# claforte/RayTracingWeekend.jl

Measured on AMD Instinct MI355X. Metric: Msamples/s (pixels x spp) on scene_random_spheres 1920x1080, higher is better.
Workload: dtype f32

## Files before the change

### raytracingweekend.jl_amd/csrc/rtw_host.hpp

```cpp
#pragma once
#pragma GCC visibility push(default)
#include "../../include/rtw_hip.h"
#pragma GCC visibility pop

#include <hip/hip_runtime.h>

#include <algorithm>
#include <atomic>
#include <cmath>
#include <cstdarg>
#include <cstddef>
#include <cstdint>
#include <cstdio>
#include <cstdlib>
#include <cstring>
#include <initializer_list>
#include <limits>
#include <map>
#include <memory>
#include <mutex>
#include <string>
#include <thread>
#include <type_traits>
#include <vector>
// ... 1 lines not shown
#pragma GCC visibility push(hidden)

#include "rtw_layout.hpp"

namespace rtw { struct DevCounters; }


struct rtw_scene_dev {
    int device;
    int is_f64;
    int n, n_pad;
    void *geom, *mat0, *mat1;
    void *scan;
    void *mf_ops;
    int mf_blocks;
    float mf_sc, mf_sigma2, mf_oo_keep, mf_o1_coef, mf_o_max;
    int n_huge, huge[2];
    void *p_mf_ops, *p_geom, *p_mat0, *p_mat1;
    unsigned short *p_orig;
    int p_alias, p_n, p_n_pad, p_mf_blocks, p_huge[2];
    void *c_mf_ops, *c_mf_box;
    float c_glo[3], c_ghi[3];
    int c_mf_blocks;
    float c_grid[6];
    int c_n_inlane, c_inlane[8];
    void *c_bound, *c_exact, *c_mat0, *c_mat1;
    unsigned short *c_orig;
    int c_groups_pad, c_big;
    double c_cs[3], c_rs;
    uint64_t content_hash;
};
// ... 285 lines not shown
```

### raytracingweekend.jl_amd/csrc/rtw_launch.hip

```cpp
#include "rtw_scene_view.hpp"
#include "rtw_kernels.hpp"
#include "rtw_instances.hpp"
#ifdef RTW_WITH_POOL
#include "rtw_pool.hpp"
template <typename T> using pool_kern_t = void (*)(rtw::KParams, rtw::Camera<T>, rtw::DevScene<T>, T *, rtw::DevCounters *);
#endif

namespace rtwh {

void make_udiv(unsigned d, unsigned *m, unsigned *s) {
    if (d <= 1) { *m = 0; *s = 0x80000000u; return; }
    unsigned l = 0;
    while ((1ull << l) < d) ++l;
    *m = (unsigned)((((1ull << l) - d) << 32) / d + 1);
    *s = l - 1;
}

struct PoolChoice { bool use = false; const void *kern = nullptr; size_t lds = 0; int block_threads = 256, blocks_per_cu = 0; };
template <typename T>
static int choose_pool(const DeviceCtx *ctx, const rtw_scene_dev *scene, const rtw_params *p, int cs, bool eligible, bool phase_profile, PoolChoice *pool) {
#ifdef RTW_WITH_POOL
    static const bool env_pool = aid_flag("RTW_POOL");
    if constexpr (sizeof(T) == 4) {
        pool->lds = rtw::pool_fixed_lds_bytes<T, RTW_POOL_W, RTW_POOL_R>() + rtw::pool_scene_lds_bytes<T>(scene->n, scene->n_pad);
// ... 238 lines not shown
    } else if (aid_env("RTW_PHASE_PROFILE")) {
        double tot = 0;
        for (int k = 0; k < 6; ++k) tot += (double)c.phase[k];
        fprintf(stderr, "[rtw phase profile] wave-cycles: pull %.1f%%  sample+scatter finish %.1f%%  scan-pass1/level1 %.1f%%  extract/level2 %.1f%%  resolve %.1f%%  shade %.1f%%  (total %.3g)\n",
                100 * c.phase[0] / tot, 100 * c.phase[1] / tot, 100 * c.phase[2] / tot, 100 * c.phase[4] / tot,
                100 * c.phase[5] / tot, 100 * c.phase[3] / tot, tot);
        if (c.phase[8])
            fprintf(stderr, "[rtw phase profile] lane loop: %llu wave-iterations, lane utilisation at the scan %.2f %% (%llu lanes with a ray), %.2f %% of the iterations without any ray; "
                            "lane-iterations lost at batch boundaries %.2f %% (pool short) + %.2f %% (no usable batch)\n", (unsigned long long)c.phase[8],
                    100.0 * (double)c.phase[9] / (64.0 * (double)c.phase[8]), (unsigned long long)c.phase[9], 100.0 * (double)c.phase[10] / (double)c.phase[8],
                    100.0 * (double)c.phase[11] / (64.0 * (double)c.phase[8]), 100.0 * (double)c.phase[12] / (64.0 * (double)c.phase[8]));
        if (c.phase[8]) {
            fprintf(stderr, "[rtw phase counts] per wave-iteration:");
            static const char *nm[32] = {0, 0, 0, 0, 0, 0, "blocks_without_candidate", "blocks", "iterations", "lanes_with_ray", "iterations_without_ray", "takers_pool_short", "takers_unserved",
                                         "list_entries", "exact_test_rounds", "exact_tests", "reject_trials", "R_executed", "H1_executed", "H1_rounds", "A_executed", "jobs_stored", "batches_set_up",
                                         "H2_executed", "B_executed", "F_normalize_executed", "sign_collections", "blocks_recording", "explode_iterations", "reject_trials_3_draws", 0, 0};
            for (int k = 6; k < 32; ++k) if (nm[k]) fprintf(stderr, " %s=%.4f", nm[k], (double)c.phase[k] / (double)c.phase[8]);
            fprintf(stderr, "\n");
        }
        if (c.phase[8] && c.phase[13])
            fprintf(stderr, "[rtw phase profile] pass 2: %.1f list entries, %.2f exact-test rounds and %.1f exact tests per wave-iteration (lanes busy in a round: %.1f %%)\n",
                    (double)c.phase[13] / (double)c.phase[8], (double)c.phase[14] / (double)c.phase[8], (double)c.phase[15] / (double)c.phase[8], 100.0 * (double)c.phase[15] / (64.0 * (double)c.phase[14]));
        if (c.phase[7])
            fprintf(stderr, "[rtw phase profile] matrix-pipe scan: %.1f%% of the (wave, block of 32 spheres) evaluations found no candidate in any lane (%llu of %llu)\n",
                    100.0 * (double)c.phase[6] / (double)c.phase[7], (unsigned long long)c.phase[6], (unsigned long long)c.phase[7]);
    }
    if (r->ctr_bytes == sizeof(rtw::DevCounters) && c.end_hist[0] == 0xdeadbeefu) {
        fprintf(stderr, "[rtw pool watchdog]");
        for (int k = 1; k <= 113; ++k) fprintf(stderr, " %u", c.end_hist[k]);
        fprintf(stderr, "\n");
    }
// ... 32 lines not shown
```

### raytracingweekend.jl_amd/csrc/rtw_probes.hpp

```cpp
#pragma once

#ifdef RTW_DUP_OPERANDS
#define RTW_PROBE_OPERANDS_TWICE()                                                                                                          \
    {                                                                                                                                       \
        float ox2 = ox, oy2 = oy, oz2 = oz, dx2_ = dx, dy2_ = dy, dz2_ = dz;                                                                \
        __asm__ volatile("" : "+v"(ox2), "+v"(oy2), "+v"(oz2), "+v"(dx2_), "+v"(dy2_), "+v"(dz2_));                                         \
        const float q_ = __builtin_fmaf(oz2, dz2_, __builtin_fmaf(oy2, dy2_, ox2 * dx2_));                                                  \
        const float oo_ = __builtin_fmaf(oz2, oz2, __builtin_fmaf(oy2, oy2, ox2 * ox2));                                                    \
        const float o1_ = (__builtin_fabsf(ox2) + __builtin_fabsf(oy2)) + __builtin_fabsf(oz2);                                             \
        const float oop_ = __builtin_fmaf(oo_, w.mf_oo_keep, -(w.mf_o1_coef * o1_));                                                        \
        const float tq_ = w.mf_sigma2 * __builtin_fmaf(q_, q_, -oop_);                                                                      \
        const float fp_[3] = {__builtin_fmaf(-q_, dx2_, ox2) * zs2, __builtin_fmaf(-q_, dy2_, oy2) * zs2, __builtin_fmaf(-q_, dz2_, oz2) * zs2}; \
        const float ax_ = dx2_ * z2, ay_ = dy2_ * z2, az_ = dz2_ * z2;                                                                      \
        const float fq_[6] = {ax_ * dx2_, ay_ * dy2_, az_ * dz2_, (ax_ + ax_) * dy2_, (ax_ + ax_) * dz2_, (ay_ + ay_) * dz2_};              \
        unsigned sq_[6], sp_[3];                                                                                                            \
        for (int k = 0; k < 6; ++k) sq_[k] = split_f16(fq_[k]);                                                                             \
        for (int k = 0; k < 3; ++k) sp_[k] = split_f16(fp_[k]);                                                                             \
        const float tx_ = ok ? tq_ : tx;                                                                                                    \
        const _Float16 t1_ = (_Float16)(tx_ * (1.0f / 32768.0f));                                                                           \
        const unsigned x23_ = split_f16((tx_ - 32768.0f * (float)t1_) * (1.0f / 16.0f));                                                    \
        const unsigned a0[8] = {dup(sq_[0]), cat(sq_[0], sq_[1]), sq_[1], dup(sq_[2]), sq_[5], dup(sp_[0]), cat(sp_[0], sp_[1]), sp_[1]};   \
        const unsigned a1[8] = {cat(sq_[2], sq_[3]), sq_[3], dup(sq_[4]), cat(sq_[4], sq_[5]), dup(sp_[2]), cat(sp_[2], sb),                \
                                ss | ((unsigned)__builtin_bit_cast(unsigned short, t1_) << 16), x23_};                                      \
        for (int k = 0; k < 8; ++k) {                                                                                                       \
            const auto sw2 = __builtin_amdgcn_permlane32_swap(a0[k], a1[k], false, false);                                                  \
            __asm__ volatile("" :: "v"(sw2[0]), "v"(sw2[1]));                                                                               \
        }                                                                                                                                   \
    }
#else
#define RTW_PROBE_OPERANDS_TWICE()
#endif

#ifdef RTW_PROBE_NO_MFMA
#define RTW_PROBE_FILTER_PAIR_REPLACED(a1, a2, b1, b2)                                                                                      \
    {                                                                                                                                       \
        rtw_f16v Wn = {-1, -1, -1, -1, -1, -1, -1, -1, -1, -1, -1, -1, -1, -1, -1, -1};                                                     \
        const uint4 u1 = __builtin_bit_cast(uint4, b1), u2 = __builtin_bit_cast(uint4, b2);                                                 \
        __asm__ volatile("" :: "v"(a1.x), "v"(a1.y), "v"(a1.z), "v"(a1.w), "v"(a2.x), "v"(a2.y), "v"(a2.z), "v"(a2.w));                     \
// ... 70 lines not shown
```

### raytracingweekend.jl_amd/csrc/rtw_scan.hpp

```cpp
#pragma once
#include "rtw_path.hpp"

namespace rtw {

#define RTW_SPHERE_WORD 32
#define RTW_SPHERE_TAIL 8
__host__ __device__ inline int scene_geom_alloc(int n, int n_pad) {
    const int a = n_pad + RTW_SPHERE_TAIL, b = ((n + 31) / 32) * 32;
    return a > b ? a : b;
}
template <typename T> struct DevScene {
    const float *scan;
    const typename Vec4<T>::type *geom;
    const typename Vec4<T>::type *mat0;
    const typename Vec4<T>::type *mat1;
    int n, n_pad;
    const uint4 *mf_ops;
    int mf_blocks;
    float mf_sc;
    float mf_sigma2;
    float mf_oo_keep;
    float mf_o1_coef;
    float mf_o_max;
    int n_huge, huge[2];
    int numerics;
    const unsigned short *orig;
};

#define RTW_LIST_CAP 16
#define RTW_LDS_SCENE_MAX_BYTES (24 * 1024)

__device__ __forceinline__ uint32_t sign_word(float x) { return __float_as_uint(x); }
__device__ __forceinline__ uint32_t sign_word(double x) { return (uint32_t)((uint64_t)__double_as_longlong(x) >> 32); }

#ifndef RTW_SCAN_PRIO
#define RTW_SCAN_PRIO 1
#endif
template <typename T> struct ScanGroup;
// ... 175 lines not shown
```

### raytracingweekend.jl_amd/csrc/rtw_scan_mfma.hpp

```cpp
#pragma once
#include "rtw_scan.hpp"
#include "rtw_cull_tables.hpp"
#include "rtw_probes.hpp"

namespace rtw {

#define RTW_PAIR_CAP 512
typedef _Float16 rtw_h8 __attribute__((ext_vector_type(8)));
typedef float rtw_f16v __attribute__((ext_vector_type(16)));

__host__ __device__ inline int cull_tab_words(int blocks) { return ((blocks + 31) / 32 > 0 ? (blocks + 31) / 32 : 1) * RTW_CULL_TAB_WORDS; }
struct CullGrid {
    float inv[3], off[3];
};

struct MfmaCull {
    const uint4 *ops;
    const float *box;
    int blocks;
    float cs[3], rs;
    const void *mat0;
    float glo[3], ghi[3];
    int n_huge;
    int n_exact;
// ... 17 lines not shown
__device__ __forceinline__ float lane_get(float v, unsigned src_lane) {
    return __int_as_float(__builtin_amdgcn_ds_bpermute((int)(src_lane << 2), __float_as_int(v)));
}
__device__ __forceinline__ double lane_get(double v, unsigned src_lane) {
    const long long b = __double_as_longlong(v);
    const unsigned lo = (unsigned)__builtin_amdgcn_ds_bpermute((int)(src_lane << 2), (int)(unsigned)b);
    const unsigned hi = (unsigned)__builtin_amdgcn_ds_bpermute((int)(src_lane << 2), (int)(unsigned)((unsigned long long)b >> 32));
    return __longlong_as_double((long long)(((unsigned long long)hi << 32) | lo));
}

#ifndef RTW_INLANE_FILTER
#define RTW_INLANE_FILTER 1
#endif
#ifndef RTW_PRECHECK_GROUPS
#define RTW_PRECHECK_GROUPS 1
#endif
#ifndef RTW_SCAN_SKIP
#define RTW_SCAN_SKIP 1
#endif

struct NoOrig {};
template <typename T, bool WITH_R, typename SRC, typename ORIG = NoOrig, typename SINK = NoSink>
__device__ __forceinline__ void test_singles(int num, SRC src, [[maybe_unused]] const typename Vec4<T>::type *rad, V3<T> o, V3<T> d, T tmin, const WaveScratch &ws, const unsigned *singles, unsigned n, unsigned lane, ORIG orig, unsigned *prof, [[maybe_unused]] SINK sink = SINK()) {
    constexpr bool CULLED = !__is_same(ORIG, NoOrig);
    using V4 = typename Vec4<T>::type;
    for (unsigned p0 = 0; p0 < n; p0 += 64u) {
        const unsigned p = p0 + lane;
        const bool valid = p < n;
        const unsigned e = singles[valid ? p : 0u];
        if (prof) { prof[0] += 1u; prof[1] += (unsigned)__popcll(__ballot(valid)); }
// ... 62 lines not shown
    __builtin_amdgcn_wave_barrier();
}

template <typename T, typename SRC, typename RAD, typename ORIG = NoOrig, typename SINK = NoSink>
__device__ __forceinline__ void resolve_pairs(int num, SRC src, RAD rad, V3<T> o, V3<T> d, T tmin, const WaveScratch &ws, unsigned n, unsigned lane, ORIG orig = ORIG(), unsigned *prof = nullptr, SINK sink = SINK()) {
    if (num == NUM_REFERENCE_FMA2) resolve_pairs_impl<T, true>(num, src, rad(), o, d, tmin, ws, n, lane, orig, prof, sink);
    else resolve_pairs_impl<T, false>(num, src, nullptr, o, d, tmin, ws, n, lane, orig, prof, sink);
}

template <typename T, typename SRC, typename ORIG = NoOrig, typename CLK = NoClock, typename SINK = NoSink, bool VOTE = !__is_same(ORIG, NoOrig)>
__device__ __forceinline__ int hit_world_mfma(const DevScene<T> &w, SRC src, V3<T> o, V3<T> d, bool has_ray, T tmin, T &t_hit,
                                              const WaveScratch &ws, unsigned lane, CLK &&clk = NoClock(),
                                              const MfmaCull *mc = nullptr, ORIG orig = ORIG(), SINK sink = SINK()) {
    constexpr bool HAS_ORIG = !__is_same(ORIG, NoOrig);
    constexpr bool CULLED = VOTE;
    static_assert(HAS_ORIG || !VOTE, "the group cull's order comes with its index array");
    auto rad = [&]() -> const typename Vec4<T>::type * { if constexpr (CULLED) return (const typename Vec4<T>::type *)mc->mat0; else return w.mat0; };
    const float ox = (float)o.x, oy = (float)o.y, oz = (float)o.z, dx = (float)d.x, dy = (float)d.y, dz = (float)d.z;
    const float s2 = __builtin_fmaf(dz, dz, __builtin_fmaf(dy, dy, dx * dx));
    const float oinf = __builtin_fmaxf(__builtin_fmaxf(__builtin_fabsf(ox), __builtin_fabsf(oy)), __builtin_fabsf(oz));
    const bool ok = has_ray && s2 <= 1.0009f && oinf <= w.mf_o_max;
    if constexpr (SINK::on()) { if (has_ray) sink.ray(lane, ok, w.mf_sc); }
    const float q = __builtin_fmaf(oz, dz, __builtin_fmaf(oy, dy, ox * dx));
    const float oo = __builtin_fmaf(oz, oz, __builtin_fmaf(oy, oy, ox * ox));
    const float o1 = (__builtin_fabsf(ox) + __builtin_fabsf(oy)) + __builtin_fabsf(oz);
    const float oop = __builtin_fmaf(oo, w.mf_oo_keep, -(w.mf_o1_coef * o1));
    const float tq = w.mf_sigma2 * __builtin_fmaf(q, q, -oop);
    const float z = ok ? 1.0f : 0.0f, z2 = z + z, zs2 = z2 * w.mf_sc;
    const float fp[3] = {__builtin_fmaf(-q, dx, ox) * zs2, __builtin_fmaf(-q, dy, oy) * zs2, __builtin_fmaf(-q, dz, oz) * zs2};
    const float dx2 = dx * z2, dy2 = dy * z2, dz2 = dz * z2;
// ... 45 lines not shown
        mine = (cells_ok ? mine : 0u) | t[flag_word];
        mine |= (unsigned)__builtin_amdgcn_update_dpp(0, (int)mine, 0xB1, 0xf, 0xf, true);
        mine |= (unsigned)__builtin_amdgcn_update_dpp(0, (int)mine, 0x4E, 0xf, 0xf, true);
        mine |= (unsigned)__builtin_amdgcn_update_dpp(0, (int)mine, 0x141, 0xf, 0xf, true);
        mine |= (unsigned)__builtin_amdgcn_update_dpp(0, (int)mine, 0x140, 0xf, 0xf, true);
        v0_ = (unsigned)__builtin_amdgcn_readlane((int)mine, 0) | (unsigned)__builtin_amdgcn_readlane((int)mine, 16);
        v1_ = (unsigned)__builtin_amdgcn_readlane((int)mine, 32) | (unsigned)__builtin_amdgcn_readlane((int)mine, 48);
    };
    uint4 A1 = {0u, 0u, 0u, 0u}, A2 = {0u, 0u, 0u, 0u};
    auto fetch = [&](int b) {
        typedef unsigned u4 __attribute__((ext_vector_type(4)));
        const __attribute__((address_space(1))) u4 *q = (const __attribute__((address_space(1))) u4 *)pa_of(b);
        __asm__("" : "+s"(q));
        A1 = __builtin_bit_cast(uint4, q[(size_t)lane]); A2 = __builtin_bit_cast(uint4, q[(size_t)lane + 64u]);
    };
    if constexpr (!CULLED) fetch(0);
    unsigned sq[6], sp[3];
#pragma unroll
    for (int k = 0; k < 6; ++k) sq[k] = split_f16(fq[k]);
#pragma unroll
    for (int k = 0; k < 3; ++k) sp[k] = split_f16(fp[k]);
    const _Float16 t1 = (_Float16)(tx * (1.0f / 32768.0f));
    const float trem = tx - 32768.0f * (float)t1;
    const unsigned x23 = split_f16(trem * (1.0f / 16.0f));
    const unsigned sb = ok ? 0x7800u : 0u, ss = ok ? 0x4c00u : 0u;
    auto dup = [](unsigned v) { return __builtin_amdgcn_perm(v, v, 0x01000100u); };
    auto cat = [](unsigned a, unsigned b) { return __builtin_amdgcn_alignbit(b, a, 16); };
    const unsigned g0[8] = {dup(sq[0]), cat(sq[0], sq[1]), sq[1], dup(sq[2]),
                            sq[5], dup(sp[0]), cat(sp[0], sp[1]), sp[1]};
    const unsigned g1[8] = {cat(sq[2], sq[3]), sq[3], dup(sq[4]), cat(sq[4], sq[5]),
                            dup(sp[2]), cat(sp[2], sb), ss | ((unsigned)__builtin_bit_cast(unsigned short, t1) << 16), x23};
    unsigned h0[8], h1[8];
#pragma unroll
    for (int k = 0; k < 8; ++k) {
        const auto sw = __builtin_amdgcn_permlane32_swap(g0[k], g1[k], false, false);
        h0[k] = sw[0]; h1[k] = sw[1];
    }
    RTW_PROBE_OPERANDS_TWICE();
    rtw_h8 B1[2], B2[2];
    {
        const uint4 q10 = {h0[0], h0[1], h0[2], h0[3]}, q11 = {h1[0], h1[1], h1[2], h1[3]};
        const uint4 q20 = {h0[4], h0[5], h0[6], h0[7]}, q21 = {h1[4], h1[5], h1[6], h1[7]};
        B1[0] = __builtin_bit_cast(rtw_h8, q10); B1[1] = __builtin_bit_cast(rtw_h8, q11);
        B2[0] = __builtin_bit_cast(rtw_h8, q20); B2[1] = __builtin_bit_cast(rtw_h8, q21);
    }
    const unsigned lane_const = lane << 16;
// ... 112 lines not shown
            }
            return any;
        };
        [[maybe_unused]] auto eval = [&](const rtw_f16v &Wv, unsigned &bits) {
#pragma unroll
            for (int r = 0; r < 16; ++r) bits = __builtin_amdgcn_alignbit(bits, __float_as_uint(Wv[r]), 31);
        };
        auto filter_pair = [&](const uint4 &a1, const uint4 &a2, const rtw_h8 &b1, const rtw_h8 &b2) -> rtw_f16v {
            RTW_PROBE_FILTER_PAIR_REPLACED(a1, a2, b1, b2);
            rtw_f16v Wp = __builtin_amdgcn_mfma_f32_32x32x16_f16(__builtin_bit_cast(rtw_h8, a1), b1, zero, 0, 0, 0);
            Wp = __builtin_amdgcn_mfma_f32_32x32x16_f16(__builtin_bit_cast(rtw_h8, a2), b2, Wp, 0, 0, 0);
            RTW_PROBE_FILTER_PAIR_AGAIN(Wp, a1, a2, b1, b2);
            return Wp;
        };
        unsigned long long some0 = 0ull, some1 = 0ull;
        if (!CULLED || do_half0) {
            rtw_f16v Wv = filter_pair(A1, A2, B1[0], B2[0]);
            RTW_PROBE_EVAL_TWICE(Wv);
            some0 = collect(Wv, bits);
        }
        if (!CULLED || do_half1) {
            rtw_f16v Wv = filter_pair(A1, A2, B1[1], B2[1]);
            __builtin_amdgcn_sched_barrier(0);
            fetch(blk);
            __builtin_amdgcn_sched_barrier(0);
            RTW_PROBE_EVAL_TWICE(Wv);
            some1 = collect(Wv, bits);
        } else {
            fetch(blk);
        }
        clk.lap(2);
        if constexpr (!CULLED) clk.count(7, 1u);
        if (RTW_SCAN_SKIP && !(some0 | some1)) {
            if constexpr (!CULLED) clk.count(6, 1u);
        } else {
        unsigned long long got1 = some1;
        __asm__("" : "+s"(got1));
        const unsigned m = ~bits << (got1 ? 0u : 16u);
        if constexpr (!CULLED) { if (!__any(m != 0u)) clk.count(6, 1u); }
        const unsigned long long act = __ballot(m != 0u);
        clk.count(27, 1u);
        if (total + 64u > ws.cap) {
            clk.lap(4);
            if constexpr (SINK::on()) sink.flush(lane, RTW_FLUSH_A);
// ... 36 lines not shown
```

### raytracingweekend.jl_amd/csrc/rtw_scene.hip

```cpp
#include "rtw_scene_view.hpp"
#include "rtw_cull_tables.hpp"
#include "rtw_plain_layout.hpp"

namespace rtwh {

template <typename SceneT>
void kd_split(const SceneT *s, std::vector<int> &ids, int lo, int hi, std::vector<std::vector<int>> &groups) {
    const int cnt = hi - lo;
    if (cnt <= RTW_CULL_GS) {
        if (cnt > 0) groups.emplace_back(ids.begin() + lo, ids.begin() + hi);
        return;
    }
    double mn[3] = {1e300, 1e300, 1e300}, mx[3] = {-1e300, -1e300, -1e300};
    for (int k = lo; k < hi; ++k) {
        const double c[3] = {(double)s->cx[ids[k]], (double)s->cy[ids[k]], (double)s->cz[ids[k]]};
        for (int a = 0; a < 3; ++a) { mn[a] = std::min(mn[a], c[a]); mx[a] = std::max(mx[a], c[a]); }
    }
    int ax = 0;
    for (int a = 1; a < 3; ++a) if (mx[a] - mn[a] > mx[ax] - mn[ax]) ax = a;
    const int unit = cnt > 2 * RTW_CULL_GS ? 2 * RTW_CULL_GS : RTW_CULL_GS;
    int half = ((cnt / 2 + unit - 1) / unit) * unit;
    if (half >= cnt) half = cnt - 1;
    auto key = [&](int i) { return ax == 0 ? (double)s->cx[i] : ax == 1 ? (double)s->cy[i] : (double)s->cz[i]; };
    std::nth_element(ids.begin() + lo, ids.begin() + lo + half, ids.begin() + hi, [&](int a, int b) { return key(a) < key(b); });
// ... 155 lines not shown

template <typename T, typename V4>
int build_mfma_operands(const std::vector<V4> &geom, int n, rtw_scene_dev *h, void **ops_out, int *blocks_out, int n_skip, const int *skip, int n_rows) {
    *ops_out = nullptr; *blocks_out = 0;
    if (n <= 0) return 0;
    auto live = [&](int i) { return i < n && (double)geom[i].w > -1e29; };
    if (n_rows < 0) n_rows = n;
    auto in_filter = [&](int i) { if (!live(i) || i >= n_rows) return false; for (int k = 0; k < n_skip; ++k) if (skip[k] == i) return false; return true; };
    double emax = 0;
    for (int i = 0; i < n; ++i) {
        if (!live(i)) continue;
        const double r = std::sqrt(std::fabs((double)geom[i].w));
        emax = std::max(emax, std::max(std::max(std::fabs((double)(float)geom[i].x), std::fabs((double)(float)geom[i].y)),
                                       std::max(std::fabs((double)(float)geom[i].z), r)));
    }
    if (!(emax > 0) || !std::isfinite(emax)) return 0;
    int ex = 0;
    (void)std::frexp(emax, &ex);
    if (ex > 40 || ex < -40) return 0;
    const double sc = std::ldexp(1.0, 8 - ex), sig2 = sc * sc;
    const double phi_c = std::ldexp(1.0, -25) / sc, phi_k = std::ldexp(1.0, -20) / sig2;
    const double A_S = std::ldexp(1.0, -17), A_r = std::ldexp(12.0, -22);
    auto split = [](double x, unsigned &p1, unsigned &p2) {
        const float xf = (float)x;
        const _Float16 h1 = (_Float16)xf;
        const _Float16 h2 = (_Float16)(xf - (float)h1);
        unsigned short b1, b2;
        memcpy(&b1, &h1, 2); memcpy(&b2, &h2, 2);
        p1 = b1; p2 = b2;
    };
    const int nb = (n_rows + 31) / 32;
    std::vector<uint4> ops((size_t)(nb + 1) * 128);
    for (int blk = 0; blk <= nb; ++blk)
        for (int lane = 0; lane < 64; ++lane) {
            const int i = lane & 31, H = lane >> 5;
            const int sph = blk * 32 + 16 * ((i >> 2) & 1) + (((i >> 3) << 2) | (i & 3));
            double fq[6] = {0, 0, 0, 0, 0, 0}, fl[3] = {0, 0, 0};
            double kx = -1073741824.0;
            if (in_filter(sph)) {
                const double cx = (double)(float)geom[sph].x, cy = (double)(float)geom[sph].y, cz = (double)(float)geom[sph].z;
                const double r2 = (double)geom[sph].w, c2 = cx * cx + cy * cy + cz * cz;
                const double Gs = 1.02 * ((2 * A_S + A_r) * c2 + A_r * r2 + 9 * phi_c * (std::fabs(cx) + std::fabs(cy) + std::fabs(cz)) + 1.5 * phi_k);
                kx = (r2 - c2 + Gs) * sig2;
                const double hs = 0.5 * sig2;
                fq[0] = cx * cx * hs; fq[1] = cy * cy * hs; fq[2] = cz * cz * hs; fq[3] = cx * cy * hs; fq[4] = cx * cz * hs; fq[5] = cy * cz * hs;
                fl[0] = cx * sc; fl[1] = cy * sc; fl[2] = cz * sc;
            }
            unsigned q1[6], q2[6], l1[3], l2[3];
            for (int k = 0; k < 6; ++k) split(fq[k], q1[k], q2[k]);
            for (int k = 0; k < 3; ++k) split(fl[k], l1[k], l2[k]);
            const _Float16 k1 = (_Float16)(float)(kx / 32768.0);
            const double rem = (kx - 32768.0 * (double)(float)k1) / 16.0;
            _Float16 k2 = (_Float16)(float)rem;
            if ((double)(float)k2 < rem) { unsigned short b; memcpy(&b, &k2, 2); b = (unsigned short)((float)k2 >= 0.0f ? b + 1 : b - 1); memcpy(&k2, &b, 2); }
            unsigned short kb1, kb2;
            memcpy(&kb1, &k1, 2); memcpy(&kb2, &k2, 2);
            auto pk = [](unsigned lo, unsigned hi) { return (lo & 0xffffu) | (hi << 16); };
            uint4 m1, m2;
            if (H == 0) {
                m1 = uint4{pk(q1[0], q2[0]), pk(q1[0], q1[1]), pk(q2[1], q1[1]), pk(q1[2], q2[2])};
                m2 = uint4{pk(q2[5], q1[5]), pk(l1[0], l2[0]), pk(l1[0], l1[1]), pk(l2[1], l1[1])};
            } else {
                m1 = uint4{pk(q1[2], q1[3]), pk(q2[3], q1[3]), pk(q1[4], q2[4]), pk(q1[4], q1[5])};
                m2 = uint4{pk(l1[2], l2[2]), pk(l1[2], kb1), pk(kb2, 0x7800u), 0x4c004c00u};
            }
            ops[(size_t)blk * 128 + lane] = m1;
            ops[(size_t)blk * 128 + 64 + lane] = m2;
        }
    HIP_TRY(hipMalloc(ops_out, ops.size() * sizeof(uint4)));
    HIP_TRY(hipMemcpy(*ops_out, ops.data(), ops.size() * sizeof(uint4), hipMemcpyHostToDevice));
    *blocks_out = nb;
    h->mf_sc = (float)sc; h->mf_sigma2 = (float)sig2;
    float keep = (float)(1.0 - 1.02 * 2 * A_S);
    if ((double)keep > 1.0 - 1.02 * 2 * A_S) keep = std::nextafter(keep, 0.0f);
    h->mf_oo_keep = keep;
    float coef = (float)(1.02 * 9 * phi_c);
    if ((double)coef < 1.02 * 9 * phi_c) coef = std::nextafter(coef, INFINITY);
    h->mf_o1_coef = coef;
    h->mf_o_max = (float)(std::ldexp(1.0, 13) / sc);
    return 0;
}

template <typename T, typename V4>
int build_plain(const std::vector<V4> &geom, const std::vector<V4> &mat0, const std::vector<V4> &mat1, int n, rtw_scene_dev *h) {
    if (!h->mf_ops) return 0;
    static const bool keep_env = aid_env("RTW_PLAIN_ORDER") != nullptr && strcmp(aid_env("RTW_PLAIN_ORDER"), "caller") == 0;
    auto is_huge = [&](int i) { for (int k = 0; k < h->n_huge; ++k) if (h->huge[k] == i) return true; return false; };
    std::vector<int> filt;
    std::vector<double> cx, cy, cz;
    for (int i = 0; i < n; ++i) {
        if (is_huge(i)) continue;
        filt.push_back(i);
        cx.push_back((double)geom[i].x); cy.push_back((double)geom[i].y); cz.push_back((double)geom[i].z);
    }
// ... 140 lines not shown
```

### raytracingweekend.jl_amd/csrc/rtw_scene_view.hpp

```cpp
#pragma once
#include "rtw_host.hpp"
#include "rtw_device.hpp"

namespace rtwh {

template <typename T>
rtw::CullScene<T> cull_scene_of(const rtw_scene_dev *h) {
    using V4 = typename rtw::Vec4<T>::type;
    rtw::CullScene<T> C;
    C.box = (const T *)h->c_bound; C.exact = (const V4 *)h->c_exact; C.orig = h->c_orig;
    C.mat0 = (const V4 *)h->c_mat0; C.mat1 = (const V4 *)h->c_mat1;
    C.n_groups_pad = h->c_groups_pad; C.n_big = h->c_big;
    C.cs[0] = (T)h->c_cs[0]; C.cs[1] = (T)h->c_cs[1]; C.cs[2] = (T)h->c_cs[2]; C.rs = (T)h->c_rs;
    C.kappa = sizeof(T) == 4 ? (T)0.00390625 : (T)2.384185791015625e-07;
    C.mf_ops = (const uint4 *)h->c_mf_ops; C.mf_box = (const float *)h->c_mf_box; C.mf_blocks = h->c_mf_blocks;
    for (int k = 0; k < 3; ++k) { C.mf_glo[k] = h->c_glo[k]; C.mf_ghi[k] = h->c_ghi[k]; }
    static_assert(RTW_CULL_INLANE_MAX == 8, "rtw_scene_dev::c_inlane");
    C.n_huge = h->c_mf_ops ? h->c_n_inlane : 0;
    C.n_huge_exact = h->c_mf_ops ? std::min(h->n_huge, h->c_n_inlane) : 0;
    for (int k = 0; k < 3; ++k) { C.grid.inv[k] = h->c_grid[k]; C.grid.off[k] = h->c_grid[3 + k]; }
    C.numerics = rtw::NUM_REFERENCE;
    return C;
}

template <typename T>
rtw::DevScene<T> dev_scene_of(const rtw_scene_dev *h) {
    using V4 = typename rtw::Vec4<T>::type;
    rtw::DevScene<T> S;
    memset(&S, 0, sizeof S);
    S.geom = (const V4 *)h->geom; S.mat0 = (const V4 *)h->mat0; S.mat1 = (const V4 *)h->mat1;
    S.scan = (const float *)(h->scan ? h->scan : h->geom);
    S.n = h->n; S.n_pad = h->n_pad;
    S.mf_ops = (const uint4 *)h->mf_ops; S.mf_blocks = h->mf_blocks;
    S.mf_sc = h->mf_sc; S.mf_sigma2 = h->mf_sigma2; S.mf_oo_keep = h->mf_oo_keep; S.mf_o1_coef = h->mf_o1_coef; S.mf_o_max = h->mf_o_max;
    S.n_huge = h->mf_ops ? h->n_huge : 0; S.huge[0] = h->huge[0]; S.huge[1] = h->huge[1];
    return S;
}

template <typename T>
rtw::DevScene<T> dev_scene_plain_of(const rtw_scene_dev *h) {
    using V4 = typename rtw::Vec4<T>::type;
    rtw::DevScene<T> S = dev_scene_of<T>(h);
    S.geom = (const V4 *)h->p_geom; S.mat0 = (const V4 *)h->p_mat0; S.mat1 = (const V4 *)h->p_mat1;
    S.n = h->p_n; S.n_pad = h->p_n_pad;
    S.mf_ops = (const uint4 *)h->p_mf_ops; S.mf_blocks = h->p_mf_blocks;
    S.huge[0] = h->p_huge[0]; S.huge[1] = h->p_huge[1];
    S.orig = h->p_orig;
    return S;
}
// ... 34 lines not shown
```

Baseline: 5792.

## Split MFMA sphere filter into coarse stage and skip refinement when decided

Reorders the f16 operand layout so the first MFMA on the high parts (with a conservative margin term mf_mr added to the threshold) gives a coarse answer. If every lane's result for a half-block is already decided negative, the second refinement MFMA and the candidate collection are skipped. This also moves the host-side operand construction into a shared header with a new margin scale. The aim is to cut matrix-pipe work per block, at the cost of a wave-wide branch, a split fetch, and a slightly looser coarse bound.

After: 6257 (median of 6 runs). 8.0% higher.

```diff
diff --git a/raytracingweekend.jl_amd/csrc/rtw_host.hpp b/raytracingweekend.jl_amd/csrc/rtw_host.hpp
--- a/raytracingweekend.jl_amd/csrc/rtw_host.hpp
+++ b/raytracingweekend.jl_amd/csrc/rtw_host.hpp
@@ -39,7 +39,7 @@
     void *scan;
     void *mf_ops;
     int mf_blocks;
-    float mf_sc, mf_sigma2, mf_oo_keep, mf_o1_coef, mf_o_max;
+    float mf_sc, mf_sigma2, mf_oo_keep, mf_o1_coef, mf_o_max, mf_mr;
     int n_huge, huge[2];
     void *p_mf_ops, *p_geom, *p_mat0, *p_mat1;
     unsigned short *p_orig;
diff --git a/raytracingweekend.jl_amd/csrc/rtw_launch.hip b/raytracingweekend.jl_amd/csrc/rtw_launch.hip
--- a/raytracingweekend.jl_amd/csrc/rtw_launch.hip
+++ b/raytracingweekend.jl_amd/csrc/rtw_launch.hip
@@ -276,7 +276,7 @@
             fprintf(stderr, "[rtw phase counts] per wave-iteration:");
             static const char *nm[32] = {0, 0, 0, 0, 0, 0, "blocks_without_candidate", "blocks", "iterations", "lanes_with_ray", "iterations_without_ray", "takers_pool_short", "takers_unserved",
                                          "list_entries", "exact_test_rounds", "exact_tests", "reject_trials", "R_executed", "H1_executed", "H1_rounds", "A_executed", "jobs_stored", "batches_set_up",
-                                         "H2_executed", "B_executed", "F_normalize_executed", "sign_collections", "blocks_recording", "explode_iterations", "reject_trials_3_draws", 0, 0};
+                                         "H2_executed", "B_executed", "F_normalize_executed", "sign_collections", "blocks_recording", "explode_iterations", "reject_trials_3_draws", "half_blocks", "half_blocks_settled_coarse"};
             for (int k = 6; k < 32; ++k) if (nm[k]) fprintf(stderr, " %s=%.4f", nm[k], (double)c.phase[k] / (double)c.phase[8]);
             fprintf(stderr, "\n");
         }
diff --git a/raytracingweekend.jl_amd/csrc/rtw_mfma_operands.hpp b/raytracingweekend.jl_amd/csrc/rtw_mfma_operands.hpp
--- /dev/null
+++ b/raytracingweekend.jl_amd/csrc/rtw_mfma_operands.hpp
@@ -0,0 +1,143 @@
+#pragma once
+#include <cmath>
+#include <cstdint>
+#include <cstring>
+
+namespace rtwh {
+
+inline double f16_rn(double x) {
+    if (x == 0.0) return x;
+    int e;
+    (void)std::frexp(std::fabs(x), &e);
+    int q = e - 11;
+    if (q < -24) q = -24;
+    return std::ldexp(std::nearbyint(std::ldexp(x, -q)), q);
+}
+inline double f16_up(double x) {
+    double h = f16_rn(x);
+    if (h < x) {
+        int e;
+        (void)std::frexp(std::fabs(h), &e);
+        int q = (h == 0.0 ? -24 : e - 11);
+        if (h < 0.0 && std::ldexp(1.0, e - 1) == -h) q -= 1;
+        if (q < -24) q = -24;
+        h += std::ldexp(1.0, q);
+    }
+    return h;
+}
+inline unsigned f16_bits(double h) {
+    if (h == 0.0) return std::signbit(h) ? 0x8000u : 0u;
+    const unsigned sign = h < 0.0 ? 0x8000u : 0u;
+    int e;
+    const double m = std::frexp(std::fabs(h), &e);
+    if (e - 1 < -14) return sign | (unsigned)std::ldexp(std::fabs(h), 24);
+    return sign | ((unsigned)(e - 1 + 15) << 10) | ((unsigned)std::ldexp(m, 11) & 0x3ffu);
+}
+inline double f16_value(unsigned b) {
+    const double sign = (b & 0x8000u) ? -1.0 : 1.0;
+    const int ex = (int)((b >> 10) & 31u), fr = (int)(b & 0x3ffu);
+    if (ex == 0) return sign * std::ldexp((double)fr, -24);
+    return sign * std::ldexp((double)(fr + 1024), ex - 25);
+}
+inline void f16_split(float x, double &p1, double &p2) {
+    p1 = f16_rn((double)x);
+    p2 = f16_rn((double)x - p1);
+}
+
+#define RTW_MF_MS_C2 (1.01 * (1.506 * 0x1p-10 + 3.1 * 0x1p-20))
+#define RTW_MF_MS_R2 (1.01 * 1.1 * 0x1p-20)
+#define RTW_MF_MS_FLOOR 0x1p-19
+#define RTW_MF_MR_O2 (1.01 * (0.502 * 0x1p-10 + 1.003 * 0x1p-11 + 2.1 * 0x1p-20))
+#define RTW_MF_MR_FLOOR 0x1p-9f
+struct MfmaScales {
+    double sc, sig2, phi_c, phi_k;
+    float keep, coef, o_max, mr;
+};
+inline bool mfma_scales(double emax, MfmaScales *S) {
+    if (!(emax > 0) || !std::isfinite(emax)) return false;
+    int ex = 0;
+    (void)std::frexp(emax, &ex);
+    if (ex > 40 || ex < -40) return false;
+    S->sc = std::ldexp(1.0, 8 - ex); S->sig2 = S->sc * S->sc;
+    S->phi_c = std::ldexp(1.0, -25) / S->sc; S->phi_k = std::ldexp(1.0, -20) / S->sig2;
+    const double A_S = std::ldexp(1.0, -17);
+    float keep = (float)(1.0 - 1.02 * 2 * A_S);
+    if ((double)keep > 1.0 - 1.02 * 2 * A_S) keep = std::nextafter(keep, 0.0f);
+    S->keep = keep;
+    float coef = (float)(1.02 * 9 * S->phi_c);
+    if ((double)coef < 1.02 * 9 * S->phi_c) coef = std::nextafter(coef, INFINITY);
+    S->coef = coef;
+    S->o_max = (float)(std::ldexp(1.0, 13) / S->sc);
+    float mr = (float)(RTW_MF_MR_O2 * S->sig2);
+    if ((double)mr < RTW_MF_MR_O2 * S->sig2) mr = std::nextafter(mr, INFINITY);
+    S->mr = mr;
+    return true;
+}
+
+struct MfmaSphereRow { double q1[6], q2[6], l1[3], l2[3], k1, k2, kx; };
+inline void mfma_sphere_row(bool in_filter, double cx, double cy, double cz, double r2, const MfmaScales &S, MfmaSphereRow *R) {
+    double fq[6] = {0, 0, 0, 0, 0, 0}, fl[3] = {0, 0, 0};
+    double kx = -1073741824.0, fold = 0.0;
+    if (in_filter) {
+        const double c2 = cx * cx + cy * cy + cz * cz;
+        const double A_S = std::ldexp(1.0, -17), A_r = std::ldexp(12.0, -22);
+        const double Gs = 1.02 * ((2 * A_S + A_r) * c2 + A_r * r2 + 9 * S.phi_c * (std::fabs(cx) + std::fabs(cy) + std::fabs(cz)) + 1.5 * S.phi_k);
+        kx = (r2 - c2 + Gs) * S.sig2;
+        fold = (RTW_MF_MS_C2 * c2 + RTW_MF_MS_R2 * r2) * S.sig2 + RTW_MF_MS_FLOOR;
+        const double hs = 0.5 * S.sig2;
+        fq[0] = cx * cx * hs; fq[1] = cy * cy * hs; fq[2] = cz * cz * hs; fq[3] = cx * cy * hs; fq[4] = cx * cz * hs; fq[5] = cy * cz * hs;
+        fl[0] = cx * S.sc; fl[1] = cy * S.sc; fl[2] = cz * S.sc;
+    }
+    for (int k = 0; k < 6; ++k) f16_split((float)fq[k], R->q1[k], R->q2[k]);
+    for (int k = 0; k < 3; ++k) f16_split((float)fl[k], R->l1[k], R->l2[k]);
+    R->kx = kx;
+    R->k1 = f16_up((kx + fold) / 32768.0);
+    R->k2 = f16_up((kx - 32768.0 * R->k1) / 16.0);
+}
+inline void mfma_sphere_words(const MfmaSphereRow &R, int H, uint32_t m1[4], uint32_t m2[4]) {
+    auto pk = [](double lo, double hi) { return (uint32_t)(f16_bits(lo) | (f16_bits(hi) << 16)); };
+    if (H == 0) {
+        m1[0] = pk(R.q1[0], R.q1[1]); m1[1] = pk(R.q1[2], R.q1[3]); m1[2] = pk(R.q1[4], R.q1[5]); m1[3] = pk(R.l1[1], R.l2[1]);
+        m2[0] = pk(R.q2[0], R.q1[0]); m2[1] = pk(R.q2[1], R.q1[1]); m2[2] = pk(R.q2[2], R.q1[2]); m2[3] = pk(R.q2[3], R.q1[3]);
+    } else {
+        m1[0] = pk(R.l2[0], R.l1[0]); m1[1] = pk(R.l2[2], R.l1[2]); m1[2] = pk(R.l1[0], R.l1[2]); m1[3] = pk(R.k1, 32768.0);
+        m2[0] = pk(R.q2[4], R.q1[4]); m2[1] = pk(R.q2[5], R.q1[5]); m2[2] = pk(R.l1[1], R.k2); m2[3] = pk(16.0, 16.0);
+    }
+}
+
+struct MfmaRayWords { uint32_t g0[8], g1[8]; bool ok; float tx; };
+inline void mfma_ray_words(const float o[3], const float d[3], bool has_ray, const MfmaScales &S, MfmaRayWords *Wd) {
+    const float ox = o[0], oy = o[1], oz = o[2], dx = d[0], dy = d[1], dz = d[2];
+    const float sc = (float)S.sc, sig2 = (float)S.sig2;
+    const float s2 = std::fmaf(dz, dz, std::fmaf(dy, dy, dx * dx));
+    const float oinf = std::fmax(std::fmax(std::fabs(ox), std::fabs(oy)), std::fabs(oz));
+    const bool ok = has_ray && s2 <= 1.0009f && oinf <= S.o_max;
+    const float q = std::fmaf(oz, dz, std::fmaf(oy, dy, ox * dx));
+    const float oo = std::fmaf(oz, oz, std::fmaf(oy, oy, ox * ox));
+    const float o1 = (std::fabs(ox) + std::fabs(oy)) + std::fabs(oz);
+    const float oop = std::fmaf(oo, S.keep, -(S.coef * o1));
+    const float tq = sig2 * std::fmaf(q, q, -oop);
+    const float z = ok ? 1.0f : 0.0f, z2 = z + z, zs2 = z2 * sc;
+    const float fp[3] = {std::fmaf(-q, dx, ox) * zs2, std::fmaf(-q, dy, oy) * zs2, std::fmaf(-q, dz, oz) * zs2};
+    const float dx2 = dx * z2, dy2 = dy * z2, dz2 = dz * z2;
+    const float fq[6] = {dx2 * dx, dy2 * dy, dz2 * dz, (dx2 + dx2) * dy, (dx2 + dx2) * dz, (dy2 + dy2) * dz};
+    const float tx = ok ? tq : (has_ray ? 60000.0f * 32768.0f : -60000.0f * 32768.0f);
+    const float um = std::fmaf(oo, S.mr, RTW_MF_MR_FLOOR);
+    const float txm = tx + (ok ? um : 0.0f);
+    double q1[6], q2[6], p1[3], p2[3], t2, t3;
+    for (int k = 0; k < 6; ++k) f16_split(fq[k], q1[k], q2[k]);
+    for (int k = 0; k < 3; ++k) f16_split(fp[k], p1[k], p2[k]);
+    const double t1 = f16_rn((double)(txm * (1.0f / 32768.0f)));
+    const float trem = std::fmaf(-32768.0f, (float)t1, tx);
+    f16_split(trem * (1.0f / 16.0f), t2, t3);
+    const double big = ok ? 32768.0 : 0.0, small = ok ? 16.0 : 0.0;
+    auto pk = [](double lo, double hi) { return (uint32_t)(f16_bits(lo) | (f16_bits(hi) << 16)); };
+    const uint32_t a0[8] = {pk(q1[0], q1[1]), pk(q1[2], q1[3]), pk(q1[4], q1[5]), pk(p1[1], p1[1]),
+                            pk(q1[0], q2[0]), pk(q1[1], q2[1]), pk(q1[2], q2[2]), pk(q1[3], q2[3])};
+    const uint32_t a1[8] = {pk(p1[0], p2[0]), pk(p1[2], p2[2]), pk(p1[0], p1[2]), pk(big, t1),
+                            pk(q1[4], q2[4]), pk(q1[5], q2[5]), pk(p2[1], small), pk(t2, t3)};
+    std::memcpy(Wd->g0, a0, sizeof a0); std::memcpy(Wd->g1, a1, sizeof a1);
+    Wd->ok = ok; Wd->tx = tx;
+}
+
+}
diff --git a/raytracingweekend.jl_amd/csrc/rtw_probes.hpp b/raytracingweekend.jl_amd/csrc/rtw_probes.hpp
--- a/raytracingweekend.jl_amd/csrc/rtw_probes.hpp
+++ b/raytracingweekend.jl_amd/csrc/rtw_probes.hpp
@@ -17,11 +17,12 @@
         for (int k = 0; k < 6; ++k) sq_[k] = split_f16(fq_[k]);                                                                             \
         for (int k = 0; k < 3; ++k) sp_[k] = split_f16(fp_[k]);                                                                             \
         const float tx_ = ok ? tq_ : tx;                                                                                                    \
-        const _Float16 t1_ = (_Float16)(tx_ * (1.0f / 32768.0f));                                                                           \
-        const unsigned x23_ = split_f16((tx_ - 32768.0f * (float)t1_) * (1.0f / 16.0f));                                                    \
-        const unsigned a0[8] = {dup(sq_[0]), cat(sq_[0], sq_[1]), sq_[1], dup(sq_[2]), sq_[5], dup(sp_[0]), cat(sp_[0], sp_[1]), sp_[1]};   \
-        const unsigned a1[8] = {cat(sq_[2], sq_[3]), sq_[3], dup(sq_[4]), cat(sq_[4], sq_[5]), dup(sp_[2]), cat(sp_[2], sb),                \
-                                ss | ((unsigned)__builtin_bit_cast(unsigned short, t1_) << 16), x23_};                                      \
+        const float txm_ = tx_ + (ok ? __builtin_fmaf(oo_, w.mf_mr, 0x1p-9f) : 0.0f);                                                       \
+        const _Float16 t1_ = (_Float16)(txm_ * (1.0f / 32768.0f));                                                                          \
+        const unsigned x23_ = split_f16(__builtin_fmaf(-32768.0f, (float)t1_, tx_) * (1.0f / 16.0f));                                       \
+        const unsigned a0[8] = {lead(sq_[0], sq_[1]), lead(sq_[2], sq_[3]), lead(sq_[4], sq_[5]), dup(sp_[1]), sq_[0], sq_[1], sq_[2], sq_[3]};\
+        const unsigned a1[8] = {sp_[0], sp_[2], lead(sp_[0], sp_[2]), sb | ((unsigned)__builtin_bit_cast(unsigned short, t1_) << 16),       \
+                                sq_[4], sq_[5], cat(sp_[1], ss), x23_};                                                                     \
         for (int k = 0; k < 8; ++k) {                                                                                                       \
             const auto sw2 = __builtin_amdgcn_permlane32_swap(a0[k], a1[k], false, false);                                                  \
             __asm__ volatile("" :: "v"(sw2[0]), "v"(sw2[1]));                                                                               \
diff --git a/raytracingweekend.jl_amd/csrc/rtw_scan.hpp b/raytracingweekend.jl_amd/csrc/rtw_scan.hpp
--- a/raytracingweekend.jl_amd/csrc/rtw_scan.hpp
+++ b/raytracingweekend.jl_amd/csrc/rtw_scan.hpp
@@ -22,6 +22,7 @@
     float mf_oo_keep;
     float mf_o1_coef;
     float mf_o_max;
+    float mf_mr;
     int n_huge, huge[2];
     int numerics;
     const unsigned short *orig;
diff --git a/raytracingweekend.jl_amd/csrc/rtw_scan_mfma.hpp b/raytracingweekend.jl_amd/csrc/rtw_scan_mfma.hpp
--- a/raytracingweekend.jl_amd/csrc/rtw_scan_mfma.hpp
+++ b/raytracingweekend.jl_amd/csrc/rtw_scan_mfma.hpp
@@ -55,6 +55,9 @@
 #endif
 #ifndef RTW_PRECHECK_GROUPS
 #define RTW_PRECHECK_GROUPS 1
+#endif
+#ifndef RTW_TWO_STAGE
+#define RTW_TWO_STAGE 1
 #endif
 #ifndef RTW_SCAN_SKIP
 #define RTW_SCAN_SKIP 1
@@ -147,6 +150,7 @@
                                               const MfmaCull *mc = nullptr, ORIG orig = ORIG(), SINK sink = SINK()) {
     constexpr bool HAS_ORIG = !__is_same(ORIG, NoOrig);
     constexpr bool CULLED = VOTE;
+    constexpr bool TWO_STAGE = RTW_TWO_STAGE != 0 && !VOTE;
     static_assert(HAS_ORIG || !VOTE, "the group cull's order comes with its index array");
     auto rad = [&]() -> const typename Vec4<T>::type * { if constexpr (CULLED) return (const typename Vec4<T>::type *)mc->mat0; else return w.mat0; };
     const float ox = (float)o.x, oy = (float)o.y, oz = (float)o.z, dx = (float)d.x, dy = (float)d.y, dz = (float)d.z;
@@ -222,22 +226,30 @@
         __asm__("" : "+s"(q));
         A1 = __builtin_bit_cast(uint4, q[(size_t)lane]); A2 = __builtin_bit_cast(uint4, q[(size_t)lane + 64u]);
     };
+    [[maybe_unused]] auto fetch_row = [&](int b, uint4 &A, unsigned row) {
+        typedef unsigned u4 __attribute__((ext_vector_type(4)));
+        const __attribute__((address_space(1))) u4 *q = (const __attribute__((address_space(1))) u4 *)pa_of(b);
+        __asm__("" : "+s"(q));
+        A = __builtin_bit_cast(uint4, q[(size_t)lane + row]);
+    };
     if constexpr (!CULLED) fetch(0);
     unsigned sq[6], sp[3];
 #pragma unroll
     for (int k = 0; k < 6; ++k) sq[k] = split_f16(fq[k]);
 #pragma unroll
     for (int k = 0; k < 3; ++k) sp[k] = split_f16(fp[k]);
-    const _Float16 t1 = (_Float16)(tx * (1.0f / 32768.0f));
-    const float trem = tx - 32768.0f * (float)t1;
+    const float txm = tx + (ok ? __builtin_fmaf(oo, w.mf_mr, 0x1p-9f) : 0.0f);
+    const _Float16 t1 = (_Float16)(txm * (1.0f / 32768.0f));
+    const float trem = __builtin_fmaf(-32768.0f, (float)t1, tx);
     const unsigned x23 = split_f16(trem * (1.0f / 16.0f));
     const unsigned sb = ok ? 0x7800u : 0u, ss = ok ? 0x4c00u : 0u;
     auto dup = [](unsigned v) { return __builtin_amdgcn_perm(v, v, 0x01000100u); };
     auto cat = [](unsigned a, unsigned b) { return __builtin_amdgcn_alignbit(b, a, 16); };
-    const unsigned g0[8] = {dup(sq[0]), cat(sq[0], sq[1]), sq[1], dup(sq[2]),
-                            sq[5], dup(sp[0]), cat(sp[0], sp[1]), sp[1]};
-    const unsigned g1[8] = {cat(sq[2], sq[3]), sq[3], dup(sq[4]), cat(sq[4], sq[5]),
-                            dup(sp[2]), cat(sp[2], sb), ss | ((unsigned)__builtin_bit_cast(unsigned short, t1) << 16), x23};
+    auto lead = [](unsigned a, unsigned b) { return __builtin_amdgcn_perm(b, a, 0x05040100u); };
+    const unsigned g0[8] = {lead(sq[0], sq[1]), lead(sq[2], sq[3]), lead(sq[4], sq[5]), dup(sp[1]),
+                            sq[0], sq[1], sq[2], sq[3]};
+    const unsigned g1[8] = {sp[0], sp[2], lead(sp[0], sp[2]), sb | ((unsigned)__builtin_bit_cast(unsigned short, t1) << 16),
+                            sq[4], sq[5], cat(sp[1], ss), x23};
     unsigned h0[8], h1[8];
 #pragma unroll
     for (int k = 0; k < 8; ++k) {
@@ -380,12 +392,55 @@
             return Wp;
         };
         unsigned long long some0 = 0ull, some1 = 0ull;
+        if constexpr (TWO_STAGE) {
+        auto coarse = [&](const uint4 &a1, const rtw_h8 &b1) -> rtw_f16v {
+            clk.count(30, 1u);
+            return __builtin_amdgcn_mfma_f32_32x32x16_f16(__builtin_bit_cast(rtw_h8, a1), b1, zero, 0, 0, 0);
+        };
+        auto undecided = [&](const rtw_f16v &Wv) -> unsigned long long {
+            unsigned t = __builtin_amdgcn_bitop3_b32(__float_as_uint(Wv[0]), __float_as_uint(Wv[1]), __float_as_uint(Wv[2]), 0x80);
+#pragma unroll
+            for (int r = 3; r < 15; r += 2) t = __builtin_amdgcn_bitop3_b32(t, __float_as_uint(Wv[r]), __float_as_uint(Wv[r + 1]), 0x80);
+            t &= __float_as_uint(Wv[15]);
+            return __ballot((int)t >= 0);
+        };
+        {
+            rtw_f16v Wv = coarse(A1, B1[0]);
+            if (undecided(Wv)) {
+                __asm__ volatile("" : "+v"(Wv));
+                Wv = __builtin_amdgcn_mfma_f32_32x32x16_f16(__builtin_bit_cast(rtw_h8, A2), B2[0], Wv, 0, 0, 0);
+                some0 = collect(Wv, bits);
+            } else {
+                clk.count(31, 1u);
+            }
+        }
+        {
+            rtw_f16v Wv = coarse(A1, B1[1]);
+            __builtin_amdgcn_sched_barrier(0);
+            fetch_row(blk, A1, 0u);
+            __builtin_amdgcn_sched_barrier(0);
+            unsigned long long open1 = undecided(Wv);
+            if (open1) {
+                __asm__ volatile("" : "+v"(Wv));
+                Wv = __builtin_amdgcn_mfma_f32_32x32x16_f16(__builtin_bit_cast(rtw_h8, A2), B2[1], Wv, 0, 0, 0);
+            } else {
+                clk.count(31, 1u);
+            }
+            __builtin_amdgcn_sched_barrier(0);
+            fetch_row(blk, A2, 64u);
+            __builtin_amdgcn_sched_barrier(0);
+            __asm__ volatile("" : "+s"(open1));
+            if (open1) some1 = collect(Wv, bits);
+        }
+        } else {
         if (!CULLED || do_half0) {
+            clk.count(30, 1u);
             rtw_f16v Wv = filter_pair(A1, A2, B1[0], B2[0]);
             RTW_PROBE_EVAL_TWICE(Wv);
             some0 = collect(Wv, bits);
         }
         if (!CULLED || do_half1) {
+            clk.count(30, 1u);
             rtw_f16v Wv = filter_pair(A1, A2, B1[1], B2[1]);
             __builtin_amdgcn_sched_barrier(0);
             fetch(blk);
@@ -394,6 +449,7 @@
             some1 = collect(Wv, bits);
         } else {
             fetch(blk);
+        }
         }
         clk.lap(2);
         if constexpr (!CULLED) clk.count(7, 1u);
diff --git a/raytracingweekend.jl_amd/csrc/rtw_scene.hip b/raytracingweekend.jl_amd/csrc/rtw_scene.hip
--- a/raytracingweekend.jl_amd/csrc/rtw_scene.hip
+++ b/raytracingweekend.jl_amd/csrc/rtw_scene.hip
@@ -1,6 +1,7 @@
 #include "rtw_scene_view.hpp"
 #include "rtw_cull_tables.hpp"
 #include "rtw_plain_layout.hpp"
+#include "rtw_mfma_operands.hpp"
 
 namespace rtwh {
 
@@ -193,70 +194,28 @@
         emax = std::max(emax, std::max(std::max(std::fabs((double)(float)geom[i].x), std::fabs((double)(float)geom[i].y)),
                                        std::max(std::fabs((double)(float)geom[i].z), r)));
     }
-    if (!(emax > 0) || !std::isfinite(emax)) return 0;
-    int ex = 0;
-    (void)std::frexp(emax, &ex);
-    if (ex > 40 || ex < -40) return 0;
-    const double sc = std::ldexp(1.0, 8 - ex), sig2 = sc * sc;
-    const double phi_c = std::ldexp(1.0, -25) / sc, phi_k = std::ldexp(1.0, -20) / sig2;
-    const double A_S = std::ldexp(1.0, -17), A_r = std::ldexp(12.0, -22);
-    auto split = [](double x, unsigned &p1, unsigned &p2) {
-        const float xf = (float)x;
-        const _Float16 h1 = (_Float16)xf;
-        const _Float16 h2 = (_Float16)(xf - (float)h1);
-        unsigned short b1, b2;
-        memcpy(&b1, &h1, 2); memcpy(&b2, &h2, 2);
-        p1 = b1; p2 = b2;
-    };
+    MfmaScales S;
+    if (!mfma_scales(emax, &S)) return 0;
     const int nb = (n_rows + 31) / 32;
     std::vector<uint4> ops((size_t)(nb + 1) * 128);
     for (int blk = 0; blk <= nb; ++blk)
         for (int lane = 0; lane < 64; ++lane) {
             const int i = lane & 31, H = lane >> 5;
             const int sph = blk * 32 + 16 * ((i >> 2) & 1) + (((i >> 3) << 2) | (i & 3));
-            double fq[6] = {0, 0, 0, 0, 0, 0}, fl[3] = {0, 0, 0};
-            double kx = -1073741824.0;
-            if (in_filter(sph)) {
-                const double cx = (double)(float)geom[sph].x, cy = (double)(float)geom[sph].y, cz = (double)(float)geom[sph].z;
-                const double r2 = (double)geom[sph].w, c2 = cx * cx + cy * cy + cz * cz;
-                const double Gs = 1.02 * ((2 * A_S + A_r) * c2 + A_r * r2 + 9 * phi_c * (std::fabs(cx) + std::fabs(cy) + std::fabs(cz)) + 1.5 * phi_k);
-                kx = (r2 - c2 + Gs) * sig2;
-                const double hs = 0.5 * sig2;
-                fq[0] = cx * cx * hs; fq[1] = cy * cy * hs; fq[2] = cz * cz * hs; fq[3] = cx * cy * hs; fq[4] = cx * cz * hs; fq[5] = cy * cz * hs;
-                fl[0] = cx * sc; fl[1] = cy * sc; fl[2] = cz * sc;
-            }
-            unsigned q1[6], q2[6], l1[3], l2[3];
-            for (int k = 0; k < 6; ++k) split(fq[k], q1[k], q2[k]);
-            for (int k = 0; k < 3; ++k) split(fl[k], l1[k], l2[k]);
-            const _Float16 k1 = (_Float16)(float)(kx / 32768.0);
-            const double rem = (kx - 32768.0 * (double)(float)k1) / 16.0;
-            _Float16 k2 = (_Float16)(float)rem;
-            if ((double)(float)k2 < rem) { unsigned short b; memcpy(&b, &k2, 2); b = (unsigned short)((float)k2 >= 0.0f ? b + 1 : b - 1); memcpy(&k2, &b, 2); }
-            unsigned short kb1, kb2;
-            memcpy(&kb1, &k1, 2); memcpy(&kb2, &k2, 2);
-            auto pk = [](unsigned lo, unsigned hi) { return (lo & 0xffffu) | (hi << 16); };
-            uint4 m1, m2;
-            if (H == 0) {
-                m1 = uint4{pk(q1[0], q2[0]), pk(q1[0], q1[1]), pk(q2[1], q1[1]), pk(q1[2], q2[2])};
-                m2 = uint4{pk(q2[5], q1[5]), pk(l1[0], l2[0]), pk(l1[0], l1[1]), pk(l2[1], l1[1])};
-            } else {
-                m1 = uint4{pk(q1[2], q1[3]), pk(q2[3], q1[3]), pk(q1[4], q2[4]), pk(q1[4], q1[5])};
-                m2 = uint4{pk(l1[2], l2[2]), pk(l1[2], kb1), pk(kb2, 0x7800u), 0x4c004c00u};
-            }
+            MfmaSphereRow row;
+            if (in_filter(sph)) mfma_sphere_row(true, (double)(float)geom[sph].x, (double)(float)geom[sph].y, (double)(float)geom[sph].z, (double)geom[sph].w, S, &row);
+            else mfma_sphere_row(false, 0, 0, 0, 0, S, &row);
+            uint32_t w1[4], w2[4];
+            mfma_sphere_words(row, H, w1, w2);
+            const uint4 m1 = {w1[0], w1[1], w1[2], w1[3]}, m2 = {w2[0], w2[1], w2[2], w2[3]};
             ops[(size_t)blk * 128 + lane] = m1;
             ops[(size_t)blk * 128 + 64 + lane] = m2;
         }
     HIP_TRY(hipMalloc(ops_out, ops.size() * sizeof(uint4)));
     HIP_TRY(hipMemcpy(*ops_out, ops.data(), ops.size() * sizeof(uint4), hipMemcpyHostToDevice));
     *blocks_out = nb;
-    h->mf_sc = (float)sc; h->mf_sigma2 = (float)sig2;
-    float keep = (float)(1.0 - 1.02 * 2 * A_S);
-    if ((double)keep > 1.0 - 1.02 * 2 * A_S) keep = std::nextafter(keep, 0.0f);
-    h->mf_oo_keep = keep;
-    float coef = (float)(1.02 * 9 * phi_c);
-    if ((double)coef < 1.02 * 9 * phi_c) coef = std::nextafter(coef, INFINITY);
-    h->mf_o1_coef = coef;
-    h->mf_o_max = (float)(std::ldexp(1.0, 13) / sc);
+    h->mf_sc = (float)S.sc; h->mf_sigma2 = (float)S.sig2;
+    h->mf_oo_keep = S.keep; h->mf_o1_coef = S.coef; h->mf_o_max = S.o_max; h->mf_mr = S.mr;
     return 0;
 }
 
diff --git a/raytracingweekend.jl_amd/csrc/rtw_scene_view.hpp b/raytracingweekend.jl_amd/csrc/rtw_scene_view.hpp
--- a/raytracingweekend.jl_amd/csrc/rtw_scene_view.hpp
+++ b/raytracingweekend.jl_amd/csrc/rtw_scene_view.hpp
@@ -32,7 +32,7 @@
     S.scan = (const float *)(h->scan ? h->scan : h->geom);
     S.n = h->n; S.n_pad = h->n_pad;
     S.mf_ops = (const uint4 *)h->mf_ops; S.mf_blocks = h->mf_blocks;
-    S.mf_sc = h->mf_sc; S.mf_sigma2 = h->mf_sigma2; S.mf_oo_keep = h->mf_oo_keep; S.mf_o1_coef = h->mf_o1_coef; S.mf_o_max = h->mf_o_max;
+    S.mf_sc = h->mf_sc; S.mf_sigma2 = h->mf_sigma2; S.mf_oo_keep = h->mf_oo_keep; S.mf_o1_coef = h->mf_o1_coef; S.mf_o_max = h->mf_o_max; S.mf_mr = h->mf_mr;
     S.n_huge = h->mf_ops ? h->n_huge : 0; S.huge[0] = h->huge[0]; S.huge[1] = h->huge[1];
     return S;
 }
```
